# PolyU-IOR/HPR-LP-C

Hardware: AMD Instinct MI355X
Metric: HPR iterations/sec (FP64) (higher is better)
Workload: dtype f64

## Files before the change

### hpr-lp-c_amd/csrc/kernels.hip

```cpp
#include "kernels.h"
#include "group_table.h"
#include "values_body.h"

#include <algorithm>
#include <array>
#include <cstring>
#include <tuple>
#include <stdexcept>
#include <vector>
#include <cmath>
#include <type_traits>

namespace hprlp {

__device__ __forceinline__ double wave_sum(double v) {
#pragma unroll
    for (int off = 32; off > 0; off >>= 1) v += __shfl_xor(v, off, kWave);
    return v;
}

__device__ __forceinline__ double wave_max(double v) {
#pragma unroll
    for (int off = 32; off > 0; off >>= 1) v = fmax(v, __shfl_xor(v, off, kWave));
    return v;
// ... 403 lines not shown
                __builtin_amdgcn_sched_barrier(0);
            }
            if (j + ED >= 0) {
                issue_entries(E[(j + ED) % ED], seg + j + ED);
                __builtin_amdgcn_sched_barrier(0);
            }
        }
        constexpr int U = (ED * TD) % 2 == 0 && ED * TD > 2 ? ED * TD : 2 * ED * TD;
        static_assert(U % ED == 0 && U % TD == 0, "the unrolled body must return every register set to its role");
        bool done = false;
        for (int k = seg; !done;) {
#pragma unroll
            for (int u = 0; u < U; ++u) {
                step(E[u % ED], tl[u % TD], k);
                if (++k >= lim) {
                    done = true;
                    break;
                }
            }
        }
    }
    if (STAMP && tid == 0) {
#pragma unroll
        for (int i = 0; i < 7; ++i) stamp[i] += ph[i];
    }
}

template <int K>
__device__ __forceinline__ void remainder_steps(const TiledDev &t, int smid, int s1, double *acc, double *prod, double *bnd, int tid) {
    constexpr int NT = kTileThreads, NW = kTileThreads / 64;
    static_assert(K == 4 || K == 6 || K == 8, "code loads: one or two 16-byte loads, or two 12-byte loads, per lane");
    if (smid >= s1) return;
    const int wave = tid >> 6, lane = tid & 63;
    double *bnd_val = bnd;
    uint32_t *bnd_row = reinterpret_cast<uint32_t *>(bnd + NW);
    constexpr uint32_t NOROW = 0x10000u;
    double pv[K];
    uint32_t cv[K];
    TileStep st = t.steps[smid];
    auto issue = [&](const TileStep &z) {
        const int last = max(z.e_end - z.e_begin - 1, 0);
#pragma unroll
        for (int k = 0; k < K; ++k) pv[k] = __builtin_nontemporal_load(t.P + z.e_begin + min(tid + k * NT, last));
        const int c0 = min(K * tid, max(last + 1 - K, 0));
        if constexpr (K == 6) {
            typedef uint32_t u3_t __attribute__((ext_vector_type(3), aligned(4)));
            const u3_t w0 = __builtin_nontemporal_load(reinterpret_cast<const u3_t *>(t.rq + z.e_begin + c0));
            const u3_t w1 = __builtin_nontemporal_load(reinterpret_cast<const u3_t *>(t.rq + z.e_begin + c0 + 3));
            cv[0] = w0.x; cv[1] = w0.y; cv[2] = w0.z; cv[3] = w1.x; cv[4] = w1.y; cv[5] = w1.z;
        } else {
            typedef uint32_t u4_t __attribute__((ext_vector_type(4), aligned(4)));
            const u4_t w0 = __builtin_nontemporal_load(reinterpret_cast<const u4_t *>(t.rq + z.e_begin + c0));
            cv[0] = w0.x; cv[1] = w0.y; cv[2] = w0.z; cv[3] = w0.w;
            if constexpr (K == 8) {
                const u4_t w1 = __builtin_nontemporal_load(reinterpret_cast<const u4_t *>(t.rq + z.e_begin + c0 + 4));
                cv[4] = w1.x; cv[5] = w1.y; cv[6] = w1.z; cv[7] = w1.w;
            }
        }
    };
    issue(st);
    for (int s = smid; s < s1; ++s) {
        const int cnt = st.e_end - st.e_begin;
        const TileStep nxt = t.steps[min(s + 1, s1 - 1)];
        lds_barrier();
#pragma unroll
        for (int k = 0; k < K; ++k) {
            const int el = tid + k * NT;
            if (el < cnt) prod[el] = pv[k];
        }
        uint32_t code[K];
        {
            const int shift = K * tid - min(K * tid, max(cnt - K, 0));
#pragma unroll
            for (int u = 0; u < K; ++u) code[u] = cv[u];
            if (shift > 0 && shift < K) {
#pragma unroll
                for (int u = 0; u < K; ++u) {
                    uint32_t c = 0;
#pragma unroll
                    for (int q = 0; q < K; ++q) c = (q == u + shift) ? cv[q] : c;
                    code[u] = c;
                }
            }
        }
        if (s + 1 < s1) issue(nxt);
        lds_barrier();
        const int nv = min(max(cnt - K * tid, 0), K);
        uint32_t row[K];
        double pr[K];
#pragma unroll
        for (int u = 0; u < K; ++u) {
            const bool ok = u < nv;
            row[u] = ok ? (code[u] & 0xffffu) : (u == 0 ? NOROW : row[u - 1]);
            pr[u] = ok ? prod[code[u] >> 16] : 0.0;
        }
        double run = pr[0], head = 0.0;
        bool single = true;
#pragma unroll
        for (int u = 1; u < K; ++u) {
            if (row[u] != row[u - 1]) {
                if (single) {
                    head = run;
                    single = false;
                } else {
                    acc[row[u - 1]] += run;
                }
                run = pr[u];
            } else {
                run += pr[u];
            }
        }
        const uint32_t rf = row[0], rl = row[K - 1];
        const uint32_t rl_prev = __shfl_up(rl, 1, 64);
        const bool open_in = lane > 0 && rf == rl_prev && rf != NOROW;
        double v = run;
        int f = (single && open_in) ? 0 : 1;
#pragma unroll
        for (int off = 1; off < 64; off <<= 1) {
            const double vu = __shfl_up(v, off, 64);
            const int fu = __shfl_up(f, off, 64);
            if (lane >= off && !f) {
                v += vu;
                f |= fu;
            }
        }
        const double v_prev = __shfl_up(v, 1, 64);
        const double carry = open_in ? v_prev : 0.0;
        const int next_open = __shfl_down(static_cast<int>(open_in), 1, 64);
        if (!single) acc[rf] += carry + head;
        const double tail = single ? carry + run : run;
        if (lane == 63) {
            bnd_row[wave] = rl;
            bnd_val[wave] = tail;
        } else if (!next_open && rl != NOROW) {
            acc[rl] += tail;
        }
        lds_barrier();
        if (tid < NW) {
            const uint32_t rw = bnd_row[tid];
            bool last_one = rw != NOROW;
            double tot = 0.0;
#pragma unroll
            for (int w = 0; w < NW; ++w) {
                const bool same = bnd_row[w] == rw;
                if (w <= tid && same) tot += bnd_val[w];
                if (w > tid && same) last_one = false;
            }
            if (last_one) acc[rw] += tot;
        }
        st = nxt;
    }
}

template <class Epi, bool PUSH>
__device__ __forceinline__ void epilogue_rows(const Epi &epi, double *acc, double (&racc)[Epi::NACC > 0 ? Epi::NACC : 1], int r0, int nr, int tid) {
    constexpr int NT = kTileThreads, B = 4;
    for (int i0 = tid; i0 < nr; i0 += B * NT) {
        typename Epi::Row rw[B];
        double sv[B][1];
#pragma unroll
        for (int u = 0; u < B; ++u) {
            const int i = min(i0 + u * NT, nr - 1);
            rw[u] = epi.load_row(r0 + i);
            sv[u][0] = acc[i];
        }
#pragma unroll
        for (int u = 0; u < B; ++u) {
            const int i = i0 + u * NT;
            if (i < nr) {
                if constexpr (PUSH) acc[i] = epi.apply(r0 + i, rw[u], sv[u], racc);
                else epi.apply(r0 + i, rw[u], sv[u], racc);
            }
        }
    }
}

__device__ __forceinline__ void push_products(const FarPush &f, const double *vals, int pb, int pe, int tid) {
    constexpr int NT = kTileThreads, U = 4;
    if (pb >= pe) return;
    double a4[U];
    int p4[U];
    uint16_t c4[U];
    auto load_batch = [&](int k0) {
#pragma unroll
        for (int u = 0; u < U; ++u) {
            const int z = min(k0 + u * NT, pe - 1);
            a4[u] = __builtin_nontemporal_load(f.val + z);
            p4[u] = __builtin_nontemporal_load(f.pos + z);
            c4[u] = __builtin_nontemporal_load(f.lcol + z);
        }
    };
    int k = pb + tid;
    load_batch(k);
    for (; k < pe; k += U * NT) {
        double prd[U];
        int ps[U];
#pragma unroll
        for (int u = 0; u < U; ++u) {
            prd[u] = a4[u] * vals[c4[u]];
            ps[u] = p4[u];
        }
        const int kn = k + U * NT;
        if (kn < pe) load_batch(kn);
#pragma unroll
        for (int u = 0; u < U; ++u)
            if (k + u * NT < pe) f.P[ps[u]] = prd[u];
    }
}

__device__ __forceinline__ int run_position(const int *tab_k, const int *tab_p, int nr, int k) {
    int lo = 0, hi = nr - 1;
    while (lo < hi) {
        const int mid = (lo + hi + 1) >> 1;
        if (tab_k[mid] <= k) lo = mid;
        else hi = mid - 1;
    }
    return tab_p[lo] + (k - tab_k[lo]);
}

__device__ __forceinline__ void push_products_runs(const FarPush &f, const double *vals, int *tab, int g, int pb, int pe, int tid) {
    constexpr int NT = kTileThreads, U = 4;
    if (pb >= pe) return;
    const int r0 = f.rptr[g], nr = f.rptr[g + 1] - r0;
    int *tab_k = tab, *tab_p = tab + kPbRunTabCap;
    double a4[U];
    uint16_t c4[U];
    auto load_batch = [&](int k0) {
#pragma unroll
        for (int u = 0; u < U; ++u) {
            const int z = min(k0 + u * NT, pe - 1);
            a4[u] = __builtin_nontemporal_load(f.val + z);
            c4[u] = __builtin_nontemporal_load(f.lcol + z);
        }
    };
    int k = pb + tid;
    load_batch(k);
    for (int i = tid; i < nr; i += NT) {
        tab_k[i] = f.rk[r0 + i];
        tab_p[i] = f.rp[r0 + i];
    }
    lds_barrier();
    int ps[U];
#pragma unroll
    for (int u = 0; u < U; ++u) ps[u] = run_position(tab_k, tab_p, nr, min(k + u * NT, pe - 1));
    for (; k < pe; k += U * NT) {
        double prd[U];
        int pc[U];
#pragma unroll
        for (int u = 0; u < U; ++u) {
            prd[u] = a4[u] * vals[c4[u]];
            pc[u] = ps[u];
        }
        const int kn = k + U * NT;
        if (kn < pe) load_batch(kn);
#pragma unroll
        for (int u = 0; u < U; ++u)
            if (k + u * NT < pe) f.P[pc[u]] = prd[u];
        if (kn < pe) {
#pragma unroll
            for (int u = 0; u < U; ++u) ps[u] = run_position(tab_k, tab_p, nr, min(kn + u * NT, pe - 1));
        }
    }
}

template <class Epi, bool REP, bool PUSH = false, bool NARROW = false>
__global__ void __launch_bounds__(kTileThreads, 4) k_tiled_fused(CsrDev A, Epi epi) {
    static_assert(Epi::NV == 1, "the tiled kernel stages one gathered vector");
    constexpr int NT = kTileThreads, RMAX = kTileRows, T = kTileCols;
    constexpr int NACC = Epi::NACC;
    __shared__ double acc[RMAX];
    __shared__ __attribute__((aligned(16))) double ytile[T];
    const TiledDev &t = A.tiled;
    const int tid = threadIdx.x;
    const int R = t.R;
    const int per = t.per, slots = gridDim.x / 8;
    const int slot = blockIdx.x / 8;
    double racc[NACC > 0 ? NACC : 1];
#pragma unroll
    for (int i = 0; i < (NACC > 0 ? NACC : 1); ++i) racc[i] = 0.0;
    epi.begin();
    int wg_round = 0;
    const bool wg_stamp = t.wgtimes && tid == 0 && (t.wg_filter == 0 || (PUSH && NACC == 0));
    if (wg_stamp) t.wgtimes[blockIdx.x * 8] = wall_clock64();
    for (int q = slot; q < per; q += slots) {
        const int sb = (blockIdx.x % 8) * per + q;
        if (sb >= t.nsb) break;
        const double *__restrict__ vec = epi.gv[0];
        lds_barrier();
        const int ncols = A.cols;
        for (int i = tid; i < R; i += NT) acc[i] = 0.0;
        const int s0 = t.sb_ptr[sb], smid = t.sb_mid[sb], s1 = t.sb_ptr[sb + 1];
        if (s0 < smid) tiled_sweep<HPRLP_SWEEP_ED, HPRLP_SWEEP_TD, REP, false, LogTerm<Epi>::value, NARROW ? kTileColsNarrow : kTileCols>(t, s0, smid - s0, t.steps[s0].rot, smid - s0, vec, ncols, acc, ytile, tid);
        remainder_steps<kTileRemK>(t, smid, s1, acc, ytile, ytile + kTileRemCap, tid);
        lds_barrier();
        const int r0 = sb * R;
        const int nr = min(R, A.rows - r0);
        int pb = 0, pe = 0;
        if constexpr (PUSH) {
            pb = epi.push.gptr[sb];
            pe = epi.push.gptr[sb + 1];
        }
        epilogue_rows<Epi, PUSH>(epi, acc, racc, r0, nr, tid);
        if constexpr (PUSH) {
            lds_barrier();
            push_products(epi.push, acc, pb, pe, tid);
        }
        if (wg_stamp && ++wg_round <= 5) t.wgtimes[blockIdx.x * 8 + wg_round] = wall_clock64();
    }
    if (wg_stamp) {
        t.wgtimes[blockIdx.x * 8 + 7] = wall_clock64();
        const unsigned hw = __builtin_amdgcn_s_getreg((31 << 11) | 4), xcc = __builtin_amdgcn_s_getreg((31 << 11) | 20);
        t.wgtimes[blockIdx.x * 8 + 6] = (static_cast<unsigned long long>(xcc & 0xfu) << 32) | hw;
    }
    if constexpr (NACC > 0) {
        __syncthreads();
        block_store_partials_in<NACC, kTileThreads / kWave, MaxAccs<Epi>::value>(racc, epi.partials, epi.stride, reinterpret_cast<double(*)[NACC]>(ytile));
    }
}

template <class Epi, bool PUSH = false>
__global__ void __launch_bounds__(kTileThreads, 4) k_pb_fused(CsrDev A, Epi epi) {
    static_assert(Epi::NV == 1, "one gathered vector");
    constexpr int NT = kTileThreads, K = kPbRemK, CAP = kPbRemCap, NW = kTileThreads / 64;
    constexpr int NACC = Epi::NACC;
// ... 168 lines not shown
    const int w = min(G, ncols - c0);
    constexpr int U = 4;
    double a[U];
    int pos[U];
    uint16_t lc[U];
    int k = b + tid;
    auto load_batch = [&](int k0) {
#pragma unroll
        for (int u = 0; u < U; ++u) {
            const int q = min(k0 + u * kFarThreads, e - 1);
            a[u] = __builtin_nontemporal_load(t.f_val + q);
            pos[u] = __builtin_nontemporal_load(t.f_pos + q);
            lc[u] = __builtin_nontemporal_load(t.f_lcol + q);
        }
    };
    load_batch(k);
    {
        constexpr int S = kFarGroup / kFarThreads;
        double sv[S];
#pragma unroll
        for (int i = 0; i < S; ++i)
            if (i * kFarThreads < G) sv[i] = vec[c0 + min(tid + i * kFarThreads, w - 1)];
#pragma unroll
        for (int i = 0; i < S; ++i)
            if (i * kFarThreads < G) v[tid + i * kFarThreads] = sv[i];
    }
    __syncthreads();
    for (; k < e; k += U * kFarThreads) {
        double pr[U];
        int ps[U];
#pragma unroll
        for (int u = 0; u < U; ++u) {
            pr[u] = LOGTERM ? a[u] - v[lc[u]] : a[u] * v[lc[u]];
            ps[u] = pos[u];
        }
        const int kn = k + U * kFarThreads;
        if (kn < e) load_batch(kn);
#pragma unroll
        for (int u = 0; u < U; ++u)
            if (k + u * kFarThreads < e) t.P[ps[u]] = pr[u];
    }
}

template <bool LOGTERM = false>
__global__ void __launch_bounds__(kFarThreads) k_far_products_runs(TiledDev t, const double *__restrict__ vec, int ncols) {
    __shared__ double v[kPbRowsMax];
    __shared__ int tab[2 * kPbRunTabCap];
    const int G = t.G;
    int g, b, e;
    if (!far_work_item(t, g, b, e)) return;
    const int c0 = g * G, tid = threadIdx.x;
    const int w = min(G, ncols - c0);
    const int r0 = t.f_rptr[g], nr = t.f_rptr[g + 1] - r0;
    int *tab_k = tab, *tab_p = tab + kPbRunTabCap;
    constexpr int U = 4;
    double a[U];
    uint16_t lc[U];
    int k = b + tid;
    auto load_batch = [&](int k0) {
#pragma unroll
        for (int u = 0; u < U; ++u) {
            const int q = min(k0 + u * kFarThreads, e - 1);
            a[u] = __builtin_nontemporal_load(t.f_val + q);
            lc[u] = __builtin_nontemporal_load(t.f_lcol + q);
        }
    };
    load_batch(k);
    for (int i = tid; i < G; i += kFarThreads) v[i] = vec[c0 + min(i, w - 1)];
    for (int i = tid; i < nr; i += kFarThreads) {
        tab_k[i] = t.f_rk[r0 + i];
        tab_p[i] = t.f_rp[r0 + i];
    }
    __syncthreads();
    int ps[U];
#pragma unroll
    for (int u = 0; u < U; ++u) ps[u] = run_position(tab_k, tab_p, nr, min(k + u * kFarThreads, e - 1));
    for (; k < e; k += U * kFarThreads) {
        double pr[U];
        int pc[U];
#pragma unroll
        for (int u = 0; u < U; ++u) {
            pr[u] = LOGTERM ? a[u] - v[lc[u]] : a[u] * v[lc[u]];
            pc[u] = ps[u];
        }
        const int kn = k + U * kFarThreads;
        if (kn < e) load_batch(kn);
#pragma unroll
        for (int u = 0; u < U; ++u)
            if (k + u * kFarThreads < e) t.P[pc[u]] = pr[u];
        if (kn < e) {
#pragma unroll
            for (int u = 0; u < U; ++u) ps[u] = run_position(tab_k, tab_p, nr, min(kn + u * kFarThreads, e - 1));
        }
    }
}

template <bool LOGTERM>
static void launch_far_products(const TiledDev &t, const double *vec, int ncols, hipStream_t s) {
    const dim3 grid(((t.f_work ? t.n_work : t.n_groups) + 7) / 8 * 8);
    if (t.f_rk && t.G <= kPbRowsMax) hipLaunchKernelGGL(k_far_products_runs<LOGTERM>, grid, dim3(kFarThreads), 0, s, t, vec, ncols);
    else hipLaunchKernelGGL(k_far_products<LOGTERM>, grid, dim3(kFarThreads), 0, s, t, vec, ncols);
}


template <bool CHECK, bool STREAMED = false>
struct XEpi {
    static constexpr int NV = 1;
    static constexpr int NACC = CHECK ? 3 : 0;
    const double *gv[1];
    double *x, *x_hat;
    const double *l, *u, *c, *last_x;
    double *x_bar, *z_bar, *x_temp;
    Ctrl *ctrl;
    double *partials;
    int stride;
    double sigma, f1, f2;
    FarPush push;
    const unsigned char *lu_code;
    int x_mode;
    double f1p, f2p;
    static constexpr bool kPublishes = true;
    static constexpr bool kSkipsX = !CHECK && STREAMED;
    struct Row {
        double xi, ci, li, ui, lx;
    };
    __device__ __forceinline__ void begin() { begin_at(blockIdx.x); }
    __device__ __forceinline__ void begin_at(int bid) {
        const int k = ctrl->kx;
        sigma = ctrl->sigma;
        f1 = 1.0 / (static_cast<double>(k) + 2.0);
        f2 = 1.0 - f1;
        f1p = 1.0 / (static_cast<double>(k - 1) + 2.0);
        f2p = 1.0 - f1p;
        if (bid == 0 && threadIdx.x == 0) ctrl->ky = k;
    }
    __device__ __forceinline__ Row load_row(int r) const {
        constexpr bool NT = STREAMED && HPRLP_EPI_NT >= 1;
        auto ld = [](const double *p) { return NT ? __builtin_nontemporal_load(p) : *p; };
        double li, ui;
        if (lu_code) {
            const unsigned cd = NT ? __builtin_nontemporal_load(lu_code + r) : lu_code[r];
            li = (cd & kLoadL) ? ld(l + r) : ((cd & kZeroL) ? 0.0 : -__builtin_huge_val());
            ui = (cd & kLoadU) ? ld(u + r) : __builtin_huge_val();
        } else {
            li = ld(l + r);
            ui = ld(u + r);
        }
        const double lx = ld(last_x + r);
        if constexpr (kSkipsX) {
            if (x_mode & kXRebuild) return Row{f2p * ld(x_hat + r) + f1p * lx, ld(c + r), li, ui, lx};
        }
        return Row{ld(x + r), ld(c + r), li, ui, lx};
    }
    __device__ __forceinline__ double apply(int r, const Row &w, const double (&s)[1], double (&acc)[CHECK ? 3 : 1]) const {
        const double gc = s[0] - w.ci;
        const double zt = w.xi + sigma * gc;
        const double xb = fmin(w.ui, fmax(w.li, zt));
        const double xh = 2.0 * xb - w.xi;
        const double xn = f2 * xh + f1 * w.lx;
        {
            if constexpr (STREAMED && HPRLP_EPI_NT >= 2) __builtin_nontemporal_store(xh, x_hat + r);
            else x_hat[r] = xh;
            if (!kSkipsX || !(x_mode & kXNoStore)) {
                if constexpr (STREAMED && HPRLP_EPI_NT >= 1) __builtin_nontemporal_store(xn, x + r);
                else x[r] = xn;
            }
        }
        if constexpr (CHECK) {
            const double zb = (xb - zt) / sigma;
            const double dx = xb - xh;
            z_bar[r] = zb;
            x_bar[r] = xb;
            x_temp[r] = dx;
            acc[0] += w.ci * xb;
            acc[1] += xb * zb;
            acc[2] += dx * dx;
        }
        return xh;
    }
};

template <bool CHECK, bool STREAMED = false>
struct YEpi {
    static constexpr int NV = 1;
    static constexpr int NACC = CHECK ? 2 : 0;
    const double *gv[1];
    double *y;
    const double *AL, *AU, *last_y;
    double *y_bar, *y_obj, *y_temp;
    Ctrl *ctrl;
    double *partials;
    int stride;
    double fact1, fact2, hf1, hf2;
    FarPush push;
    const unsigned char *row_code;
    static constexpr bool kPublishes = true;
    struct Row {
        double yi, lo, hi, ly;
    };
    __device__ __forceinline__ void begin() { begin_at(blockIdx.x); }
    __device__ __forceinline__ void begin_at(int bid) {
        const int k = ctrl->ky;
        fact1 = ctrl->lam_sigma;
        fact2 = ctrl->inv_lam_sigma;
        hf1 = 1.0 / (static_cast<double>(k) + 2.0);
        hf2 = 1.0 - hf1;
        if (bid == 0 && threadIdx.x == 0) ctrl->kx = k + 1;
    }
    __device__ __forceinline__ Row load_row(int r) const {
        constexpr bool NT = STREAMED && HPRLP_EPI_NT >= 1;
        auto ld = [](const double *p) { return NT ? __builtin_nontemporal_load(p) : *p; };
        double lo, hi;
        if (row_code) {
            const unsigned cd = NT ? __builtin_nontemporal_load(row_code + r) : row_code[r];
            hi = (cd & kLoadHi) ? ld(AU + r) : __builtin_huge_val();
            lo = (cd & kLoadLo) ? ld(AL + r) : ((cd & kRowEq) ? hi : -__builtin_huge_val());
        } else {
            lo = ld(AL + r);
            hi = ld(AU + r);
        }
        return Row{ld(y + r), lo, hi, ld(last_y + r)};
    }
    __device__ __forceinline__ double apply(int r, const Row &w, const double (&s)[1], double (&acc)[CHECK ? 2 : 1]) const {
        const double v = s[0] - fact1 * w.yi;
        const double d = fmax(w.lo - v, fmin(w.hi - v, 0.0));
        const double yb = fact2 * d;
        const double yh = 2.0 * yb - w.yi;
        const double yn = hf2 * yh + hf1 * w.ly;
        if constexpr (STREAMED && HPRLP_EPI_NT >= 2) __builtin_nontemporal_store(yn, y + r);
        else y[r] = yn;
        if constexpr (CHECK) {
            const double dy = yb - yh;
            const double yo = v + d;
            y_temp[r] = dy;
            y_bar[r] = yb;
            y_obj[r] = yo;
            acc[0] += yo * yb;
            acc[1] += dy * dy;
        }
        return yn;
    }
};

struct RdEpi {
    static constexpr int NV = 1;
    static constexpr int NACC = 1;
    const double *gv[1];
    const double *c, *z_bar, *col_norm;
    double *partials;
    int stride;
    struct Row {
        double ci, zi, cn;
    };
    __device__ __forceinline__ void begin() {}
    __device__ __forceinline__ Row load_row(int r) const { return Row{c[r], z_bar[r], col_norm[r]}; }
    __device__ __forceinline__ void apply(int, const Row &w, const double (&s)[1], double (&acc)[1]) const {
        const double rd = (w.ci - s[0] - w.zi) * w.cn;
        acc[0] += rd * rd;
    }
};

template <bool GAP>
struct RpEpi {
    static constexpr int NV = GAP ? 2 : 1;
    static constexpr int NACC = GAP ? 2 : 1;
    const double *gv[GAP ? 2 : 1];
    const double *AL, *AU, *row_norm, *y_temp;
    double *partials;
    int stride;
    struct Row {
        double lo, hi, rn, dy;
    };
    __device__ __forceinline__ void begin() {}
    __device__ __forceinline__ Row load_row(int r) const {
        return Row{AL[r], AU[r], row_norm[r], GAP ? y_temp[r] : 0.0};
    }
    __device__ __forceinline__ void apply(int, const Row &w, const double (&s)[GAP ? 2 : 1],
                                          double (&acc)[GAP ? 2 : 1]) const {
        const double v = s[0];
        const double rp = fmax(fmin(w.hi - v, 0.0), w.lo - v) * w.rn;
        acc[0] += rp * rp;
        if constexpr (GAP) acc[1] += s[1] * w.dy;
    }
};

struct GapEpi {
    static constexpr int NV = 1;
    static constexpr int NACC = 1;
    const double *gv[1];
    const double *y_temp;
    double *partials;
    int stride;
    struct Row {
        double dy;
    };
    __device__ __forceinline__ void begin() {}
    __device__ __forceinline__ Row load_row(int r) const { return Row{y_temp[r]}; }
    __device__ __forceinline__ void apply(int, const Row &w, const double (&s)[1], double (&acc)[1]) const {
        acc[0] += s[0] * w.dy;
    }
};

template <bool DOTS>
struct PlainEpi {
    static constexpr int NV = 1;
    static constexpr int NACC = DOTS ? 2 : 0;
    const double *gv[1];
    double *out;
    const double *q;
    double *partials;
    int stride;
    struct Row {
        double qi;
    };
    __device__ __forceinline__ void begin() {}
    __device__ __forceinline__ Row load_row(int r) const { return Row{DOTS ? q[r] : 0.0}; }
    __device__ __forceinline__ void apply(int r, const Row &w, const double (&s)[1], double (&acc)[DOTS ? 2 : 1]) const {
        out[r] = s[0];
        if constexpr (DOTS) {
            acc[0] += s[0] * s[0];
            acc[1] += s[0] * w.qi;
        }
    }
};

struct PlainPushEpi {
    static constexpr int NV = 1;
    static constexpr int NACC = 0;
    const double *gv[1];
    double *out;
    FarPush push;
    static constexpr bool kPublishes = true;
    struct Row {};
    __device__ __forceinline__ void begin() {}
    __device__ __forceinline__ Row load_row(int) const { return Row{}; }
    __device__ __forceinline__ double apply(int r, const Row &, const double (&s)[1], double (&)[1]) const {
        out[r] = s[0];
        return s[0];
    }
};

struct RayColEpi {
    static constexpr int NV = 1;
    static constexpr int NACC = 2;
    static constexpr int kMaxAccs = 1;
    const double *gv[1];
    const double *l, *u, *col_norm;
    double b_scale, c_scale;
    double *partials;
    int stride;
    struct Row {
        double lo, hi, cn;
    };
    __device__ __forceinline__ void begin() {}
    __device__ __forceinline__ Row load_row(int r) const { return Row{l[r], u[r], col_norm[r]}; }
    __device__ __forceinline__ void apply(int, const Row &w, const double (&s)[1], double (&acc)[2]) const {
        const double z = -((s[0] * w.cn) * c_scale);
        if (z > 0.0) {
            if (isfinite(w.lo)) acc[0] += ((w.lo / w.cn) * b_scale) * z;
            else acc[1] = fmax(acc[1], z);
        } else if (z < 0.0) {
            if (isfinite(w.hi)) acc[0] += ((w.hi / w.cn) * b_scale) * z;
            else acc[1] = fmax(acc[1], -z);
        }
    }
};

struct RayRowEpi {
    static constexpr int NV = 1;
    static constexpr int NACC = 1;
    static constexpr int kMaxAccs = 1;
    const double *gv[1];
    const double *AL, *AU, *row_norm;
    double b_scale;
    double *partials;
    int stride;
    struct Row {
        double lo, hi, rn;
    };
    __device__ __forceinline__ void begin() {}
    __device__ __forceinline__ Row load_row(int r) const { return Row{AL[r], AU[r], row_norm[r]}; }
    __device__ __forceinline__ void apply(int, const Row &w, const double (&s)[1], double (&acc)[1]) const {
        const double q = (s[0] * w.rn) * b_scale;
        if (isfinite(w.lo)) acc[0] = fmax(acc[0], -q);
        if (isfinite(w.hi)) acc[0] = fmax(acc[0], q);
    }
};

struct StartColEpi {
    static constexpr int NV = 1;
    static constexpr int NACC = 2;
    const double *gv[1];
    const double *c, *l, *u, *x_bar;
    double *z_bar;
    double *partials;
    int stride;
    struct Row {
        double ci, lo, hi, xb;
    };
    __device__ __forceinline__ void begin() {}
    __device__ __forceinline__ Row load_row(int r) const { return Row{c[r], l[r], u[r], x_bar[r]}; }
    __device__ __forceinline__ void apply(int r, const Row &w, const double (&s)[1], double (&acc)[2]) const {
        const double d = w.ci - s[0];
        const double z = ((d > 0.0 && isfinite(w.lo)) || (d < 0.0 && isfinite(w.hi))) ? d : 0.0;
        z_bar[r] = z;
        acc[0] += w.ci * w.xb;
        acc[1] += (z > 0.0 ? w.lo : (z < 0.0 ? w.hi : 0.0)) * z;
    }
};

struct StartRowEpi {
    static constexpr int NV = 1;
    static constexpr int NACC = 1;
    const double *gv[1];
    const double *AL, *AU, *y_bar;
    double *y_obj;
    double *partials;
    int stride;
    struct Row {
        double lo, hi, yb;
    };
    __device__ __forceinline__ void begin() {}
    __device__ __forceinline__ Row load_row(int r) const { return Row{AL[r], AU[r], y_bar[r]}; }
    __device__ __forceinline__ void apply(int r, const Row &w, const double (&s)[1], double (&acc)[1]) const {
        const double yo = w.yb > 0.0 ? w.lo : (w.yb < 0.0 ? w.hi : fmin(fmax(s[0], w.lo), w.hi));
        y_obj[r] = yo;
        acc[0] += yo * w.yb;
    }
};

template <class Epi>
__global__ void __launch_bounds__(kThreads) k_long_finish(CsrDev A, Epi epi, int main_grid) {
    constexpr int NV = Epi::NV;
    constexpr int NACC = Epi::NACC;
    double acc[NACC > 0 ? NACC : 1];
#pragma unroll
    for (int i = 0; i < (NACC > 0 ? NACC : 1); ++i) acc[i] = 0.0;
    epi.begin();
    const int i = blockIdx.x * kThreads + threadIdx.x;
    if (i < A.nlong) {
        const int4 d = A.longrows[i];
        double s[NV];
#pragma unroll
        for (int v = 0; v < NV; ++v) s[v] = 0.0;
        for (int c = d.y; c < d.z; ++c) {
#pragma unroll
            for (int v = 0; v < NV; ++v) s[v] += A.long_partial[static_cast<size_t>(c) * 2 + v];
        }
        typename Epi::Row rw = epi.load_row(d.x);
        epi.apply(d.x, rw, s, acc);
    }
    if constexpr (NACC > 0) {
        block_store_partials<NACC, kWavesPerBlock, MaxAccs<Epi>::value>(acc, epi.partials + main_grid, epi.stride);
    }
}

template <class Epi, class = void>
struct Publishes : std::false_type {};
template <class Epi>
struct Publishes<Epi, std::void_t<decltype(Epi::kPublishes)>> : std::true_type {};

template <class Epi>
struct WithBase : Epi {
    const double *base;
    struct Row {
        typename Epi::Row w;
        double b;
    };
    __device__ __forceinline__ Row load_row(int r) const { return Row{Epi::load_row(r), base[r]}; }
    __device__ __forceinline__ auto apply(int r, const Row &w, const double (&s)[1], double (&acc)[Epi::NACC > 0 ? Epi::NACC : 1]) const {
        const double t[1] = {w.b + s[0]};
        return Epi::apply(r, w.w, t, acc);
    }
};

struct SideEpi {
    static constexpr int NV = 1;
    static constexpr int NACC = 0;
    const double *gv[1];
    const int *rows;
    double *base;
    struct Row {};
    __device__ __forceinline__ void begin() {}
    __device__ __forceinline__ Row load_row(int) const { return Row{}; }
    __device__ __forceinline__ void apply(int r, const Row &, const double (&s)[1], double (&)[1]) const { base[rows[r]] = s[0]; }
};

template <class Epi>
static bool launch_tiled(const CsrDev &M, const Epi &e, hipStream_t s, bool far_ready);

template <class Epi>
static bool launch_fused(const CsrDev &M, const Epi &e, hipStream_t s, bool far_ready = false) {
    if (M.nblk <= 0) return false;
    if constexpr (Epi::NV == 1) {
        if (M.tiled.valid) {
            if (M.tiled.side_nblk > 0) {
                CsrDev S = M;
                S.tiled.valid = false;
                S.blk = M.tiled.side_blk;
                S.nblk = M.tiled.side_nblk;
                S.longrows = M.tiled.side_long;
                S.nlong = M.tiled.side_nlong;
                S.long_partial = M.tiled.side_partial;
                SideEpi se{{e.gv[0]}, M.tiled.side_rows, M.tiled.base};
                hipLaunchKernelGGL(k_spmv_fused<SideEpi>, dim3(S.csr_grid()), dim3(kThreads), 0, s, S, se);
                if (S.nlong > 0) hipLaunchKernelGGL(k_long_finish<SideEpi>, dim3(S.finish_grid()), dim3(kThreads), 0, s, S, se, S.csr_grid());
                WithBase<Epi> wb{e, M.tiled.base};
                return launch_tiled(M, wb, s, far_ready);
            }
            return launch_tiled(M, e, s, far_ready);
        }
    }
    hipLaunchKernelGGL(k_spmv_fused<Epi>, dim3(M.csr_grid()), dim3(kThreads), 0, s, M, e);
    if (M.nlong > 0)
        hipLaunchKernelGGL(k_long_finish<Epi>, dim3(M.finish_grid()), dim3(kThreads), 0, s, M, e, M.csr_grid());
    return false;
}

template <class Epi>
static bool launch_tiled(const CsrDev &M, const Epi &e, hipStream_t s, bool far_ready) {
    if (M.tiled.n_groups > 0 && !far_ready)
        launch_far_products<false>(M.tiled, e.gv[0], M.cols, s);
    const bool narrow = M.tiled.T == kTileColsNarrow;
    if (M.tiled.rem_cap == kPbRemCap) {
        if constexpr (Publishes<Epi>::value) {
            if (e.push.gptr) {
                hipLaunchKernelGGL((k_pb_fused<Epi, true>), dim3(M.tiled.grid), dim3(kTileThreads), 0, s, M, e);
                return true;
            }
        }
        hipLaunchKernelGGL((k_pb_fused<Epi, false>), dim3(M.tiled.grid), dim3(kTileThreads), 0, s, M, e);
        return false;
    }
    if (M.tiled.n_pieces > 0) {
        const dim3 grid((M.tiled.n_pieces + 7) / 8 * 8);
        if (narrow) hipLaunchKernelGGL((k_tiled_part<false, false, true>), grid, dim3(kTileThreads), 0, s, M, e.gv[0]);
        else if (M.tiled.stamps) hipLaunchKernelGGL((k_tiled_part<false, true>), grid, dim3(kTileThreads), 0, s, M, e.gv[0]);
        else if (M.tiled.repeats) hipLaunchKernelGGL(k_tiled_part<true>, grid, dim3(kTileThreads), 0, s, M, e.gv[0]);
        else hipLaunchKernelGGL(k_tiled_part<false>, grid, dim3(kTileThreads), 0, s, M, e.gv[0]);
        hipLaunchKernelGGL(k_tiled_finish<Epi>, dim3(M.tiled_finish_grid()), dim3(kThreads), 0, s, M, e);
        return false;
    }
    if constexpr (Publishes<Epi>::value) {
        if (e.push.gptr) {
            if (narrow) hipLaunchKernelGGL((k_tiled_fused<Epi, false, true, true>), dim3(M.tiled.grid), dim3(kTileThreads), 0, s, M, e);
            else if (M.tiled.repeats) hipLaunchKernelGGL((k_tiled_fused<Epi, true, true>), dim3(M.tiled.grid), dim3(kTileThreads), 0, s, M, e);
            else hipLaunchKernelGGL((k_tiled_fused<Epi, false, true>), dim3(M.tiled.grid), dim3(kTileThreads), 0, s, M, e);
            return true;
        }
    }
    if (narrow) hipLaunchKernelGGL((k_tiled_fused<Epi, false, false, true>), dim3(M.tiled.grid), dim3(kTileThreads), 0, s, M, e);
    else if (M.tiled.repeats) hipLaunchKernelGGL((k_tiled_fused<Epi, true>), dim3(M.tiled.grid), dim3(kTileThreads), 0, s, M, e);
    else hipLaunchKernelGGL((k_tiled_fused<Epi, false>), dim3(M.tiled.grid), dim3(kTileThreads), 0, s, M, e);
    return false;
}

FarPush far_push_of(const CsrDev &consumer) {
    FarPush f;
    if (consumer.tiled.valid && consumer.tiled.n_groups > 0) {
        f.gptr = consumer.tiled.f_gptr;
        f.val = consumer.tiled.f_val;
        f.pos = consumer.tiled.f_pos;
        f.lcol = consumer.tiled.f_lcol;
        f.P = consumer.tiled.P;
        if (consumer.tiled.f_rk) {
            f.rptr = consumer.tiled.f_rptr;
            f.rk = consumer.tiled.f_rk;
            f.rp = consumer.tiled.f_rp;
        }
    }
    return f;
}

bool launch_x_half(const CsrDev &AT, const XHalfArgs &a, bool check, hipStream_t s) {
    if (check) {
        XEpi<true> e{{a.y_full}, a.x, a.x_hat, a.l, a.u, a.c, a.last_x, a.x_bar, a.z_bar, a.x_temp, a.ctrl, a.partials, a.stride, 0, 0, 0, a.push, a.lu_code};
        return launch_fused(AT, e, s, a.far_ready);
    }
    if (AT.tiled.valid) {
        XEpi<false, true> e{{a.y_full}, a.x, a.x_hat, a.l, a.u, a.c, a.last_x, nullptr, nullptr, nullptr, a.ctrl, nullptr, 0, 0, 0, 0, a.push, a.lu_code, a.x_mode};
        return launch_fused(AT, e, s, a.far_ready);
    }
    XEpi<false> e{{a.y_full}, a.x, a.x_hat, a.l, a.u, a.c, a.last_x, nullptr, nullptr, nullptr, a.ctrl, nullptr, 0, 0, 0, 0, a.push, a.lu_code};
    return launch_fused(AT, e, s, a.far_ready);
}

bool launch_y_half(const CsrDev &A, const YHalfArgs &a, bool check, hipStream_t s) {
    if (check) {
        YEpi<true> e{{a.xhat_full}, a.y, a.AL, a.AU, a.last_y, a.y_bar, a.y_obj, a.y_temp, a.ctrl, a.partials, a.stride, 0, 0, 0, 0, a.push, a.row_code};
        return launch_fused(A, e, s, a.far_ready);
    }
    if (A.tiled.valid) {
        YEpi<false, true> e{{a.xhat_full}, a.y, a.AL, a.AU, a.last_y, nullptr, nullptr, nullptr, a.ctrl, nullptr, 0, 0, 0, 0, 0, a.push, a.row_code};
        return launch_fused(A, e, s, a.far_ready);
    }
    YEpi<false> e{{a.xhat_full}, a.y, a.AL, a.AU, a.last_y, nullptr, nullptr, nullptr, a.ctrl, nullptr, 0, 0, 0, 0, 0, a.push, a.row_code};
    return launch_fused(A, e, s, a.far_ready);
}


void launch_x_half_base(const CsrDev &AT_remote, const XHalfArgs &a, const double *base, hipStream_t s) {
    WithBase<XEpi<false>> e{{{a.y_full}, a.x, a.x_hat, a.l, a.u, a.c, a.last_x, nullptr, nullptr, nullptr, a.ctrl, nullptr, 0, 0, 0, 0, FarPush{}, a.lu_code}, base};
    launch_fused(AT_remote, e, s);
}

void launch_y_half_base(const CsrDev &A_remote, const YHalfArgs &a, const double *base, hipStream_t s) {
    WithBase<YEpi<false>> e{{{a.xhat_full}, a.y, a.AL, a.AU, a.last_y, nullptr, nullptr, nullptr, a.ctrl, nullptr, 0, 0, 0, 0, 0, FarPush{}}, base};
    launch_fused(A_remote, e, s);
}

void launch_resid_d(const CsrDev &AT, const double *ybar_full, const double *c, const double *z_bar,
                    const double *col_norm, double *partials, hipStream_t s) {
    RdEpi e{{ybar_full}, c, z_bar, col_norm, partials, AT.grid()};
    launch_fused(AT, e, s);
}

void launch_resid_p(const CsrDev &A, const double *xbar_full, const double *xtemp_full, const double *AL,
                    const double *AU, const double *row_norm, const double *y_temp, bool with_gap,
                    double *partials, int stride, hipStream_t s) {
    if (with_gap && A.tiled.valid) {
        RpEpi<false> e{{xbar_full}, AL, AU, row_norm, nullptr, partials, stride};
        launch_fused(A, e, s);
// ... 1665 lines not shown
```

Measured before the change: 771.5.

## Stage epilogue row loads with prefetched bound codes and branchless bound loads

Splits the epilogue row loading into three stages: per-row bound codes are fetched one batch ahead, unconditional loads for x/c/last_x (or y/last_y) follow, and the bound loads become branchless by redirecting unused ones to a shared row address. Scheduling barriers and empty asm uses pin the issue order so all loads of a batch are in flight together, and the next batch's codes overlap the current batch. The goal is to hide memory latency that the data-dependent conditional loads used to serialize. The cost is extra redundant loads, more registers in use, and when no code array exists the code is read as a byte from the bound array.

```diff
diff --git a/hpr-lp-c_amd/csrc/kernels.hip b/hpr-lp-c_amd/csrc/kernels.hip
--- a/hpr-lp-c_amd/csrc/kernels.hip
+++ b/hpr-lp-c_amd/csrc/kernels.hip
@@ -579,24 +579,90 @@
     }
 }
 
+template <class Epi, class = void>
+struct StagedLoads : std::false_type {};
+template <class Epi>
+struct StagedLoads<Epi, std::void_t<decltype(std::declval<const Epi &>().load_code(0))>> : std::true_type {};
+template <class T>
+__device__ __forceinline__ void needed_here(const T &v) {
+    static_assert(sizeof(T) % sizeof(double) == 0 && alignof(T) == alignof(double), "a struct of doubles");
+    double d[sizeof(T) / sizeof(double)];
+    __builtin_memcpy(d, &v, sizeof(T));
+#pragma unroll
+    for (unsigned k = 0; k < sizeof(T) / sizeof(double); ++k) asm volatile("" ::"v"(d[k]));
+}
+
 template <class Epi, bool PUSH>
 __device__ __forceinline__ void epilogue_rows(const Epi &epi, double *acc, double (&racc)[Epi::NACC > 0 ? Epi::NACC : 1], int r0, int nr, int tid) {
     constexpr int NT = kTileThreads, B = 4;
-    for (int i0 = tid; i0 < nr; i0 += B * NT) {
-        typename Epi::Row rw[B];
-        double sv[B][1];
-#pragma unroll
-        for (int u = 0; u < B; ++u) {
-            const int i = min(i0 + u * NT, nr - 1);
-            rw[u] = epi.load_row(r0 + i);
-            sv[u][0] = acc[i];
-        }
-#pragma unroll
-        for (int u = 0; u < B; ++u) {
-            const int i = i0 + u * NT;
-            if (i < nr) {
-                if constexpr (PUSH) acc[i] = epi.apply(r0 + i, rw[u], sv[u], racc);
-                else epi.apply(r0 + i, rw[u], sv[u], racc);
+    if constexpr (StagedLoads<Epi>::value) {
+        using Raw = decltype(epi.load_a(0));
+        using Sel = decltype(epi.load_b(0, 0, 0u));
+        auto issue_codes = [&](int b0, unsigned (&cd)[B]) {
+#pragma unroll
+            for (int u = 0; u < B; ++u) cd[u] = epi.load_code(r0 + min(b0 + tid + u * NT, nr - 1));
+            __builtin_amdgcn_sched_barrier(0);
+        };
+        auto batch = [&](int b0, const unsigned (&cd)[B], unsigned (&cdn)[B]) {
+            Raw ra[B];
+            Sel rs[B];
+            double sv[B][1];
+#pragma unroll
+            for (int u = 0; u < B; ++u) ra[u] = epi.load_a(r0 + min(b0 + tid + u * NT, nr - 1));
+            __builtin_amdgcn_sched_barrier(0);
+#pragma unroll
+            for (int u = 0; u < B; ++u) rs[u] = epi.load_b(r0 + min(b0 + tid + u * NT, nr - 1), r0, cd[u]);
+            __builtin_amdgcn_sched_barrier(0);
+            issue_codes(b0 + B * NT, cdn);
+#pragma unroll
+            for (int u = 0; u < B; ++u) sv[u][0] = acc[min(b0 + tid + u * NT, nr - 1)];
+#pragma unroll
+            for (int u = 0; u < B; ++u) {
+                needed_here(ra[u]);
+                needed_here(rs[u]);
+                asm volatile("" ::"v"(cdn[u]));
+            }
+            typename Epi::Row rw[B];
+#pragma unroll
+            for (int u = 0; u < B; ++u) rw[u] = epi.finish(cd[u], ra[u], rs[u]);
+#pragma unroll
+            for (int u = 0; u < B; ++u) {
+                const int i = b0 + tid + u * NT;
+                if (i < nr) {
+                    if constexpr (PUSH) acc[i] = epi.apply(r0 + i, rw[u], sv[u], racc);
+                    else epi.apply(r0 + i, rw[u], sv[u], racc);
+                }
+            }
+        };
+        if (nr <= 0) return;
+        unsigned cd0[B], cd1[B];
+        __builtin_amdgcn_sched_barrier(0);
+        issue_codes(0, cd0);
+#pragma unroll
+        for (int u = 0; u < B; ++u) asm volatile("" ::"v"(cd0[u]));
+        for (int b0 = 0;;) {
+            batch(b0, cd0, cd1);
+            if ((b0 += B * NT) >= nr) break;
+            batch(b0, cd1, cd0);
+            if ((b0 += B * NT) >= nr) break;
+        }
+    } else {
+        for (int i0 = tid; i0 < nr; i0 += B * NT) {
+            typename Epi::Row rw[B];
+            double sv[B][1];
+#pragma unroll
+            for (int u = 0; u < B; ++u) {
+                const int i = min(i0 + u * NT, nr - 1);
+                rw[u] = epi.load_row(r0 + i);
+                sv[u][0] = acc[i];
+            }
+#pragma unroll
+            for (int u = 0; u < B; ++u) {
+                const int i = i0 + u * NT;
+                if (i < nr) {
+                    if constexpr (PUSH) acc[i] = epi.apply(r0 + i, rw[u], sv[u], racc);
+                    else epi.apply(r0 + i, rw[u], sv[u], racc);
+                }
             }
         }
     }
@@ -1071,6 +1137,38 @@
         }
         return Row{ld(x + r), ld(c + r), li, ui, lx};
     }
+    struct Raw {
+        double lx, xv, ci;
+    };
+    struct Sel {
+        double lv, uv;
+    };
+    static constexpr bool kNT = STREAMED && HPRLP_EPI_NT >= 1;
+    static __device__ __forceinline__ double ld_s(const double *p) { return kNT ? __builtin_nontemporal_load(p) : *p; }
+    __device__ __forceinline__ unsigned load_code(int r) const {
+        const unsigned char *p = lu_code ? lu_code : reinterpret_cast<const unsigned char *>(l);
+        return kNT ? __builtin_nontemporal_load(p + r) : p[r];
+    }
+    __device__ __forceinline__ unsigned code_bits(unsigned loaded) const { return lu_code ? loaded : (loaded | kLoadL | kLoadU); }
+    __device__ __forceinline__ Raw load_a(int r) const {
+        const double *px = x;
+        if constexpr (kSkipsX) px = (x_mode & kXRebuild) ? x_hat : x;
+        return Raw{ld_s(last_x + r), ld_s(px + r), ld_s(c + r)};
+    }
+    __device__ __forceinline__ Sel load_b(int r, int rs, unsigned loaded) const {
+        const unsigned cd = code_bits(loaded);
+        return Sel{ld_s(l + ((cd & kLoadL) ? r : rs)), ld_s(u + ((cd & kLoadU) ? r : rs))};
+    }
+    __device__ __forceinline__ Row finish(unsigned loaded, const Raw &a, const Sel &s) const {
+        const unsigned cd = code_bits(loaded);
+        const double li = (cd & kLoadL) ? s.lv : ((cd & kZeroL) ? 0.0 : -__builtin_huge_val());
+        const double ui = (cd & kLoadU) ? s.uv : __builtin_huge_val();
+        double xi = a.xv;
+        if constexpr (kSkipsX) {
+            if (x_mode & kXRebuild) xi = f2p * a.xv + f1p * a.lx;
+        }
+        return Row{xi, a.ci, li, ui, a.lx};
+    }
     __device__ __forceinline__ double apply(int r, const Row &w, const double (&s)[1], double (&acc)[CHECK ? 3 : 1]) const {
         const double gc = s[0] - w.ci;
         const double zt = w.xi + sigma * gc;
@@ -1140,6 +1238,30 @@
         }
         return Row{ld(y + r), lo, hi, ld(last_y + r)};
     }
+    struct Raw {
+        double yi, ly;
+    };
+    struct Sel {
+        double lov, hiv;
+    };
+    static constexpr bool kNT = STREAMED && HPRLP_EPI_NT >= 1;
+    static __device__ __forceinline__ double ld_s(const double *p) { return kNT ? __builtin_nontemporal_load(p) : *p; }
+    __device__ __forceinline__ unsigned load_code(int r) const {
+        const unsigned char *p = row_code ? row_code : reinterpret_cast<const unsigned char *>(AL);
+        return kNT ? __builtin_nontemporal_load(p + r) : p[r];
+    }
+    __device__ __forceinline__ unsigned code_bits(unsigned loaded) const { return row_code ? loaded : (loaded | kLoadLo | kLoadHi); }
+    __device__ __forceinline__ Raw load_a(int r) const { return Raw{ld_s(y + r), ld_s(last_y + r)}; }
+    __device__ __forceinline__ Sel load_b(int r, int rs, unsigned loaded) const {
+        const unsigned cd = code_bits(loaded);
+        return Sel{ld_s(AL + ((cd & kLoadLo) ? r : rs)), ld_s(AU + ((cd & kLoadHi) ? r : rs))};
+    }
+    __device__ __forceinline__ Row finish(unsigned loaded, const Raw &a, const Sel &s) const {
+        const unsigned cd = code_bits(loaded);
+        const double hi = (cd & kLoadHi) ? s.hiv : __builtin_huge_val();
+        const double lo = (cd & kLoadLo) ? s.lov : ((cd & kRowEq) ? hi : -__builtin_huge_val());
+        return Row{a.yi, lo, hi, a.ly};
+    }
     __device__ __forceinline__ double apply(int r, const Row &w, const double (&s)[1], double (&acc)[CHECK ? 2 : 1]) const {
         const double v = s[0] - fact1 * w.yi;
         const double d = fmax(w.lo - v, fmin(w.hi - v, 0.0));
@@ -1387,6 +1509,19 @@
         double b;
     };
     __device__ __forceinline__ Row load_row(int r) const { return Row{Epi::load_row(r), base[r]}; }
+    template <class A>
+    struct RawB {
+        A w;
+        double b;
+    };
+    template <class E = Epi>
+    __device__ __forceinline__ auto load_code(int r) const -> decltype(this->E::load_code(r)) { return Epi::load_code(r); }
+    template <class E = Epi>
+    __device__ __forceinline__ auto load_a(int r) const -> RawB<decltype(this->E::load_a(r))> { return {Epi::load_a(r), base[r]}; }
+    template <class E = Epi>
+    __device__ __forceinline__ auto load_b(int r, int rs, unsigned cd) const -> decltype(this->E::load_b(r, rs, cd)) { return Epi::load_b(r, rs, cd); }
+    template <class A, class S>
+    __device__ __forceinline__ Row finish(unsigned cd, const RawB<A> &a, const S &s) const { return Row{Epi::finish(cd, a.w, s), a.b}; }
     __device__ __forceinline__ auto apply(int r, const Row &w, const double (&s)[1], double (&acc)[Epi::NACC > 0 ? Epi::NACC : 1]) const {
         const double t[1] = {w.b + s[0]};
         return Epi::apply(r, w.w, t, acc);
```

New measurement: 784.2 (median of 6 runs). Within noise of the previous version (+1.6%).
